# ShenhanQian/GaussianAvatars

Measured on AMD Instinct MI355X. Metric: frames/sec fwd+bwd @100k SH-3 splats 802x550, higher is better.
Workload: dtype f32; 1 GPU; BASELINE configs[2]: 100000 mesh-bound SH-3 splats (synthetic stand-in for media/306), 802x550 (HxW), select_mesh_by_timestep + render + L1-vs-white + backward, no optimiser step; splats=100000, width=550, height=802, sh_degree=3, scene=ellipsoid, splat_order=morton (io.spatial_sort: the loaders' default), num_rendered=2322054, num_binned=1851307, tile_culling=True, binding=fused, parallelism=one process, one GPU, 300 frames in turn; no collective

## Files before the change

### gaussianavatars_amd/_lib.py

```python
from __future__ import annotations

import ctypes as C
import os
from functools import partial
from typing import NamedTuple

_HERE = os.path.dirname(os.path.abspath(__file__))


def raw_stream(dev):
    import torch

    try:
        return torch._C._cuda_getCurrentRawStream(dev.index if dev.index is not None else torch.cuda.current_device())
    except AttributeError:
        return torch.cuda.current_stream(dev).cuda_stream


class _NoCtx:
    def __enter__(self):
        return None

    def __exit__(self, *a):
        return False
# ... 178 lines not shown

def gsr_profile_enable(on: bool) -> None:
    gsr().gsr_profile_enable(1 if on else 0)


def gsr_profile_read() -> dict:
    ms = (C.c_double * GSR_NUM_KERNELS)()
    n = (C.c_int64 * GSR_NUM_KERNELS)()
    rc = gsr().gsr_profile_read(ms, n)
    if rc != GSR_OK:
        raise RuntimeError(f"gsr_profile_read failed: {gsr().gsr_last_error().decode()}")
    return {gsr().gsr_kernel_name(i).decode(): (ms[i], n[i]) for i in range(GSR_NUM_KERNELS)}

def gsr_wait_stats():
    ms, n = C.c_double(), C.c_int64()
    gsr().gsr_wait_stats(C.byref(ms), C.byref(n))
    return ms.value, n.value


LIBS["gsr"] = LibSpec("gsr", GSR_LIB_PATH, GSR_SYMBOLS, GSR_ABI_VERSION)
_gsr = None


def gsr():
    global _gsr
    if _gsr is None:
        _gsr = _load(LIBS["gsr"])
    return _gsr


GAB_LIB_PATH = _lib_path("gab", "GAB_LIB")
GAB_FLAME_WS_FLOATS = 512
GAB_BIND_ROW_FLOATS = 20
_P = C.c_void_p


class GabRig(C.Structure):
    _fields_ = [("V", C.c_int32), ("n_shape", C.c_int32), ("n_expr", C.c_int32), ("v_template", _P), ("shapedirs", _P),
                ("posedirs", _P), ("J_regressor", _P), ("lbs_weights", _P), ("parents", C.c_int32 * 5)]


GAB_SYMBOLS = {
    "gab_abi_version": (C.c_int, []),
    "gab_last_error": (C.c_char_p, []),
    "gab_flame_forward": (C.c_int, [C.POINTER(GabRig)] + [_P] * 8 + [_P, _P, _P, _P]),
    "gab_flame_backward": (C.c_int, [C.POINTER(GabRig)] + [_P] * 8 + [_P, _P, _P, _P] + [_P] * 8 + [_P] +
                           [C.c_int32, C.POINTER(C.c_void_p), C.POINTER(C.c_int32), _P]),
    "gab_flame_prepared_floats": (C.c_int64, [C.POINTER(GabRig)]),
    "gab_flame_prepare": (C.c_int, [C.POINTER(GabRig), _P, _P, _P, _P]),
    "gab_flame_forward_prepared": (C.c_int, [C.POINTER(GabRig), _P] + [_P] * 6 + [_P, _P, _P, _P]),
    "gab_blend_sequence": (C.c_int, [C.POINTER(GabRig), _P, _P, C.c_int32, _P, _P]),
    "gab_flame_forward_sequence": (C.c_int, [C.POINTER(GabRig), _P, _P] + [_P] * 6 + [_P, _P, _P, _P]),
    "gab_flame_backward_prepared": (C.c_int, [C.POINTER(GabRig), _P] + [_P] * 4 + [_P, _P, _P] + [_P] * 6 + [_P] +
                                    [C.c_int32, C.POINTER(C.c_void_p), C.POINTER(C.c_int32), _P]),
    "gab_mesh_backward_prepared": (C.c_int, [C.POINTER(GabRig), _P] + [_P] * 4 + [_P, _P, _P, _P, _P] + [_P] * 5 + [_P] * 6 + [_P] +
                                   [C.c_int32, C.POINTER(C.c_void_p), C.POINTER(C.c_int32), _P]),
    "gab_face_frames_forward": (C.c_int, [C.c_int32, C.c_int32, _P, _P, C.c_int32, _P, _P, _P, _P, _P, _P]),
    "gab_face_frames_backward": (C.c_int, [C.c_int32, C.c_int32, _P, _P, C.c_int32, _P, _P, _P, _P, _P, C.c_int32, _P]),
    "gab_bind_forward": (C.c_int, [C.c_int32, C.c_int32, _P, _P, _P, _P, C.c_int32, _P, _P, _P, _P, _P, _P, _P, _P, _P, _P]),
    "gab_bind_backward": (C.c_int, [C.c_int32, C.c_int32, _P, _P, _P, _P, C.c_int32, _P, _P, _P, _P, _P, _P, _P, _P, _P, _P, _P, _P, _P, _P, _P]),
    "gab_bind_backward_csr": (C.c_int, [C.c_int32, C.c_int32] + [_P] * 22),
    "gab_bind_backward_faces": (C.c_int, [C.c_int32, _P, _P, _P, _P]),
    "gab_zero_buffers": (C.c_int, [C.c_int32, C.POINTER(C.c_void_p), C.POINTER(C.c_int32), _P]),
    "gab_feed_row": (C.c_int, [_P, C.c_int32, C.c_int32, _P, C.c_int32, _P, _P, _P]),
    **_profile_symbols("gab"),
}
GAB_ABI_VERSION = 5

LIBS["gab"] = LibSpec("gab", GAB_LIB_PATH, GAB_SYMBOLS, GAB_ABI_VERSION)
_gab = None


def gab():
    global _gab
    if _gab is None:
        _gab = _load(LIBS["gab"])
    return _gab


GLS_LIB_PATH = _lib_path("gls")
GLS_SYMBOLS = {
    "gls_abi_version": (C.c_int, []),
    "gls_last_error": (C.c_char_p, []),
    "gls_partial_floats": (C.c_int64, [C.c_int32] * 4),
    "gls_l1_ssim_forward": (C.c_int, [C.c_int32] * 4 + [_P, _P, C.c_float] + [_P] * 4),
    "gls_l1_ssim_backward": (C.c_int, [C.c_int32] * 4 + [_P] * 4 + [C.c_float, _P, _P]),
    "gls_l1_ssim_backward_split": (C.c_int, [C.c_int32] * 4 + [_P] * 5 + [C.c_int32, C.c_float, _P, _P]),
    "gls_l1_forward": (C.c_int, [C.c_int64, _P, _P, C.c_float, _P, _P, _P]),
    "gls_l1_forward_grad": (C.c_int, [C.c_int64, _P, _P, C.c_float, _P, _P, _P, _P]),
    "gls_l1_backward": (C.c_int, [C.c_int64, _P, _P, _P, C.c_float, _P, _P]),
    "gls_densification_stats": (C.c_int, [C.c_int32] + [_P] * 6),
    "gls_add_densification_stats": (C.c_int, [C.c_int32, _P, _P, C.c_int32, _P, _P, _P]),
    **_profile_symbols("gls"),
}
GLS_ABI_VERSION = 4

LIBS["gls"] = LibSpec("gls", GLS_LIB_PATH, GLS_SYMBOLS, GLS_ABI_VERSION)
_gls = None


# ... 323 lines not shown
```

### gaussianavatars_amd/binding.py

```python
from __future__ import annotations

import ctypes as C
import os

import torch

from . import _host, _lib


def _p(t):
    return None if t is None else t.data_ptr()


def _stream(dev):
    return _lib.raw_stream(dev)


def _chk(rc, what):
    if rc != 0:
        raise RuntimeError(f"{what} failed ({rc}): {_lib.gab_error()}")


def _need_cuda(t, name):
    if not t.is_cuda:
# ... 162 lines not shown
                                            _p(d_shape), _p(d_expr), _p(d_rot), _p(d_neck), _p(d_jaw), _p(d_eyes), _p(d_trans), _p(d_so),
                                            _p(scratch), 0, None, None, _stream(dev)), "gab_flame_backward")
        sh = ctx.shapes
        outs = [None, None if d_shape is None else d_shape.view(sh[0]), d_expr.view(sh[1]), d_rot.view(sh[2]), d_neck.view(sh[3]),
                d_jaw.view(sh[4]), d_eyes.view(sh[5]), d_trans.view(sh[6]), None if d_so is None else d_so.view(ctx.so_shape)]
        return tuple(outs)


def flame_forward(head, shape, expr, rotation, neck, jaw, eyes, translation, static_offset=None):
    return _FlameForward.apply(head, shape, expr, rotation, neck, jaw, eyes, translation, static_offset)


class _FlameForwardTimestep(torch.autograd.Function):

    _ROWS = ("expr", "rotation", "neck_pose", "jaw_pose", "eyes_pose", "translation")

    @staticmethod
    def forward(ctx, head, t, shape, expr, rotation, neck, jaw, eyes, translation, static_offset):
        ctx.set_materialize_grads(False)
        lib = _lib.gab()
        rig = _rig_struct(head)
        dev = head.v_template.device
        V = rig.V
        tabs = [_f32(x) for x in (expr, rotation, neck, jaw, eyes, translation)]
        T = tabs[0].shape[0]
        widths = [int(x.shape[1]) for x in tabs]
        if widths != [rig.n_expr, 3, 3, 3, 6, 3] or any(x.shape[0] != T for x in tabs) or not (0 <= t < T):
            raise RuntimeError("flame_forward_timestep: expected (T,n_expr),(T,3),(T,3),(T,3),(T,6),(T,3) tables and 0 <= t < T")
        sh = _f32(shape).reshape(-1)
        so = None if static_offset is None else _f32(static_offset).reshape(-1)
        rows = [x.data_ptr() + 4 * t * w for x, w in zip(tabs, widths)]
        verts = torch.empty((1, V, 3), dtype=torch.float32, device=dev)
        v_shaped = torch.empty((1, V, 3), dtype=torch.float32, device=dev)
        ws = torch.empty(_lib.GAB_FLAME_WS_FLOATS, dtype=torch.float32, device=dev)
        need = ctx.needs_input_grad
        ctx.prepared = _prepared_rig(head, rig, sh, so) if _use_prepared(head, need[2], so is not None and need[9]) else None
        seq = _sequence_table(head, rig, ctx.prepared, tabs[0]) if (ctx.prepared is not None and not any(need[2:])) else None
        with _lib.on_device(dev):
            if seq is not None:
                _chk(lib.gab_flame_forward_sequence(C.byref(rig), _p(ctx.prepared), seq.data_ptr() + 4 * t * 3 * V, *rows, _p(verts), _p(v_shaped),
                                                    _p(ws), _stream(dev)), "gab_flame_forward_sequence")
            elif ctx.prepared is not None:
                _chk(lib.gab_flame_forward_prepared(C.byref(rig), _p(ctx.prepared), *rows, _p(verts), _p(v_shaped), _p(ws), _stream(dev)),
                     "gab_flame_forward_prepared")
            else:
                _chk(lib.gab_flame_forward(C.byref(rig), _p(sh), *rows, _p(so), _p(verts), _p(v_shaped), _p(ws), _stream(dev)),
                     "gab_flame_forward")
        ctx.head, ctx.t, ctx.T, ctx.widths = head, t, T, widths
        ctx.has_so = so is not None
        ctx.shape_shape = shape.shape
        ctx.so_shape = None if static_offset is None else static_offset.shape
        ctx.keep = _Keep(sh, *tabs, *([so] if so is not None else []), v_shaped, ws)
        return verts, v_shaped

    @staticmethod
    def backward(ctx, g_verts, g_vshaped):
        lib = _lib.gab()
        rig = _rig_struct(ctx.head)
        saved = ctx.keep.get()
        sh, tabs = saved[0], list(saved[1:7])
        so = saved[7] if ctx.has_so else None
        v_shaped, ws = saved[-2], saved[-1]
        dev = v_shaped.device
        V, T, t, widths = rig.V, ctx.T, ctx.t, ctx.widths
        need = ctx.needs_input_grad
        f32 = dict(dtype=torch.float32, device=dev)
        tables = [torch.empty((T, w), **f32) for w in widths]
# ... 275 lines not shown
```

### gaussianavatars_amd/csrc/gaa_host.cpp

```cpp
#include <torch/extension.h>

#include <ATen/hip/impl/HIPGuardImplMasqueradingAsCUDA.h>
#include <c10/hip/HIPStream.h>
#include <dlfcn.h>
#include <torch/csrc/autograd/function.h>
#include <torch/csrc/autograd/functions/utils.h>

#include <atomic>
#include <map>
#include <mutex>
#include <tuple>

#include "../../include/gab.h"
#include "../../include/gls.h"
#include "../../include/gsr.h"

namespace {

using at::Tensor;
using torch::autograd::Node;
using torch::autograd::variable_list;

#define GAA_API(X)                                                                                                                      \
    X(gsr_abi_version) X(gsr_last_error) X(gsr_geom_layout) X(gsr_binning_layout) X(gsr_image_layout) X(gsr_forward_bound)             \
// ... 128 lines not shown
        Tensor scratch = empty_f32({3 * (int64_t)V}, v);
        Tensor gc = grad_f32(grads[2]), gR = grad_f32(grads[3]), gs = grad_f32(grads[4]), gq = grad_f32(grads[5]), gv = grad_f32(grads[0]);
        int rc = api.gab_mesh_backward_prepared(&p.rig, p.prepared.data_ptr<float>(), rows[1], rows[2], rows[3], rows[4], vs.data_ptr<float>(), ws.data_ptr<float>(),
                                                v.data_ptr<float>(), p.vf_begin.data_ptr<int32_t>(), p.vf_list.data_ptr<int32_t>(), fptr(gc), fptr(gR), fptr(gs), fptr(gq),
                                                fptr(gv), outp[0], outp[1], outp[2], outp[3], outp[4], outp[5], scratch.data_ptr<float>(), 6, zero_ptrs, zero_sizes, stream);
        TORCH_CHECK(rc == 0, "gab_mesh_backward_prepared failed (", rc, "): ", api.gab_last_error());
        variable_list out(6);
        for (int i = 0; i < 6; ++i)
            if (task_should_compute_output(i)) out[i] = tables[i];
        return out;
    }
    void release_variables() override {}
};

std::vector<Tensor> mesh_frames(const std::shared_ptr<MeshPlan>& plan, const Tensor& expr, const Tensor& rotation, const Tensor& neck, const Tensor& jaw,
                                const Tensor& eyes, const Tensor& translation, int64_t t)
{
    need_api();
    const MeshPlan& p = *plan;
    const Tensor* tabs[6] = {&expr, &rotation, &neck, &jaw, &eyes, &translation};
    const int64_t widths[6] = {p.rig.n_expr, 3, 3, 3, 6, 3};
    static const char* names[6] = {"expr", "rotation", "neck_pose", "jaw_pose", "eyes_pose", "translation"};
    const int64_t T = expr.dim() == 2 ? expr.size(0) : -1;
    TORCH_CHECK(T > 0 && t >= 0 && t < T, "flame_forward_timestep: expected (T,n_expr),(T,3),(T,3),(T,3),(T,6),(T,3) tables and 0 <= t < T");
    for (int i = 0; i < 6; ++i) {
        check_f32(*tabs[i], names[i]);
        TORCH_CHECK(tabs[i]->dim() == 2 && tabs[i]->size(0) == T && tabs[i]->size(1) == widths[i],
                    "flame_forward_timestep: expected (T,n_expr),(T,3),(T,3),(T,3),(T,6),(T,3) tables and 0 <= t < T");
    }
    const Tensor& like = p.prepared;
    DeviceGuard guard(like.device().index());
    void* stream = cur_stream(like);
    const int64_t V = p.rig.V, F = p.F;
    Tensor verts = empty_f32({1, V, 3}, like), v_shaped = empty_f32({1, V, 3}, like), ws = empty_f32({GAB_FLAME_WS_FLOATS}, like);
    Tensor center = empty_f32({F, 3}, like), R = empty_f32({F, 3, 3}, like), scale = empty_f32({F, 1}, like), quat = empty_f32({F, 4}, like);
    const float* rows[6];
    for (int i = 0; i < 6; ++i) rows[i] = tabs[i]->data_ptr<float>() + t * widths[i];
    int rc = api.gab_flame_forward_prepared(&p.rig, p.prepared.data_ptr<float>(), rows[0], rows[1], rows[2], rows[3], rows[4], rows[5], verts.data_ptr<float>(),
                                            v_shaped.data_ptr<float>(), ws.data_ptr<float>(), stream);
    TORCH_CHECK(rc == 0, "gab_flame_forward_prepared failed (", rc, "): ", api.gab_last_error());
    rc = api.gab_face_frames_forward((int32_t)V, (int32_t)F, verts.data_ptr<float>(), p.faces.data_ptr(), p.faces_i64, center.data_ptr<float>(), R.data_ptr<float>(),
                                     scale.data_ptr<float>(), quat.data_ptr<float>(), nullptr , stream);
    TORCH_CHECK(rc == 0, "gab_face_frames_forward failed (", rc, "): ", api.gab_last_error());
    if (any_requires_grad({expr, rotation, neck, jaw, eyes, translation})) {
        auto node = std::shared_ptr<MeshNode>(new MeshNode(), torch::autograd::deleteNode);
        node->set_next_edges(torch::autograd::collect_next_edges(expr, rotation, neck, jaw, eyes, translation));
        node->plan = plan;
        for (int i = 0; i < 6; ++i) {
            node->tabs[i] = Kept(*tabs[i]);
            node->widths[i] = widths[i];
        }
        node->verts = Kept(verts, true);
        node->v_shaped = Kept(v_shaped, true);
        node->ws = ws;
        node->t = t;
        node->T = T;
        torch::autograd::set_history({verts, v_shaped, center, R, scale, quat}, node);
    }
    return {verts, v_shaped, center, R, scale, quat};
}

struct Layouts {
    GsrGeomLayout geom;
    GsrImageLayout img;
};
std::mutex layout_mutex;
std::map<std::tuple<int64_t, int, int>, Layouts> layout_cache;
// ... 430 lines not shown
```

### gaussianavatars_amd/csrc/gab_kernels.hip

```cpp
#include <hip/hip_runtime.h>
#include <hip/amd_detail/amd_hip_unsafe_atomics.h>

#include "../../include/gab.h"
#include "launch_prof.h"
#include "lib_common.h"
#include "bind_math.h"
#include "wave_reduce.h"

namespace gab {

struct Rig {
    int V, n_shape, n_expr;
    const float* __restrict__ v_template;
    const float* __restrict__ shapedirs;
    const float* __restrict__ posedirs;
    const float* __restrict__ J_regressor;
    const float* __restrict__ lbs_weights;
    int parents[GAB_NUM_JOINTS];
};

constexpr int WS_J = 0;
constexpr int WS_R = 16;
constexpr int WS_PF = 64;
constexpr int WS_A = 128;
// ... 441 lines not shown
        for (int p = 0; p < GAB_POSE_FEATURES; ++p) {
            const float* row = rig.posedirs + (size_t)p * E + 3 * v;
            pf[p] = row[0] * gvp[0] + row[1] * gvp[1] + row[2] * gvp[2];
        }
    }
    const float vph[4] = {vp[0], vp[1], vp[2], ok ? 1.f : 0.f};
#pragma unroll
    for (int j = 0; j < GAB_NUM_JOINTS; ++j)
#pragma unroll
        for (int r = 0; r < 3; ++r)
#pragma unroll
            for (int c = 0; c < 4; ++c) {
                const float s = wave_sum_hi(w[j] * g[r] * vph[c]);
                if (lane == 63) red[wid][12 * j + 4 * r + c] = s;
            }
#pragma unroll
    for (int r = 0; r < 3; ++r) {
        const float s = wave_sum_hi(g[r]);
        if (lane == 63) red[wid][60 + r] = s;
    }
#pragma unroll
    for (int p = 0; p < GAB_POSE_FEATURES; ++p) {
        const float s = wave_sum_hi(pf[p]);
        if (lane == 63) red[wid][63 + p] = s;
    }
    __syncthreads();
    if (tid < 99) {
        const float s = (red[0][tid] + red[1][tid]) + (red[2][tid] + red[3][tid]);
        float* dst = tid < 60 ? &ws[WS_DA + tid] : (tid < 63 ? &ws[WS_DT + tid - 60] : &ws[WS_DPF + tid - 63]);
        unsafeAtomicAdd(dst, s);
    }
}

template <bool FLAME_TREE, int NT>
__device__ __forceinline__ void chain_bwd_body(Rig rig, float* __restrict__ ws, const float* __restrict__ rotation, const float* __restrict__ neck,
                            const float* __restrict__ jaw, const float* __restrict__ eyes, float* __restrict__ d_rotation,
                            float* __restrict__ d_neck, float* __restrict__ d_jaw, float* __restrict__ d_eyes,
                            float* __restrict__ d_translation, float* __restrict__ d_expr, float* __restrict__ d_shape,
                            const float* __restrict__ Mmat)
{
    __shared__ float sw[GAB_FLAME_WS_FLOATS];
    __shared__ float sdJ[16];
    for (int kk = threadIdx.x; kk < GAB_FLAME_WS_FLOATS; kk += NT) sw[kk] = ws[kk];
    __syncthreads();
    for (int kk = WS_DA + (int)threadIdx.x; kk < WS_DJ; kk += NT) ws[kk] = 0.f;
    if (!Mmat) {
        for (int kk = threadIdx.x; kk < rig.n_expr; kk += NT) d_expr[kk] = 0.f;
        if (d_shape)
            for (int kk = threadIdx.x; kk < rig.n_shape; kk += NT) d_shape[kk] = 0.f;
    }
    __shared__ float sdR[45];
    if (threadIdx.x == 0) {
    float J[15], R[45], Rg[45], tg[15];
#pragma unroll
    for (int k = 0; k < 15; ++k) J[k] = sw[WS_J + k];
#pragma unroll
    for (int k = 0; k < 45; ++k) R[k] = sw[WS_R + k];
    chain_forward<FLAME_TREE>(rig.parents, R, J, Rg, tg);
    float dRg[45], dtg[15], dJ[15], dR[45];
#pragma unroll
    for (int k = 0; k < 45; ++k) { dRg[k] = 0.f; dR[k] = 0.f; }
#pragma unroll
    for (int k = 0; k < 15; ++k) { dtg[k] = 0.f; dJ[k] = 0.f; }
#pragma unroll
    for (int i = 0; i < GAB_NUM_JOINTS; ++i) {
        const float* dA = sw + WS_DA + 12 * i;
#pragma unroll
        for (int r = 0; r < 3; ++r) {
            const float dAt = dA[4 * r + 3];
#pragma unroll
            for (int c = 0; c < 3; ++c) {
                dRg[9 * i + 3 * r + c] += dA[4 * r + c] - dAt * J[3 * i + c];
                dJ[3 * i + c] -= Rg[9 * i + 3 * r + c] * dAt;
            }
            dtg[3 * i + r] += dAt;
        }
    }
#pragma unroll
// ... 105 lines not shown
        if (c < nC) {
            const float* col = rig.shapedirs + (size_t)e0 * NB + c0 + c;
            int r = r0;
            for (; r + 8 <= r1; r += 8) {
                float x[8];
#pragma unroll
                for (int k = 0; k < 8; ++k) x[k] = col[(size_t)(r + k) * NB];
#pragma unroll
                for (int k = 0; k < 8; ++k) acc += x[k] * g[r + k];
            }
            for (; r < r1; ++r) acc += col[(size_t)r * NB] * g[r];
        }
        if (half == 1) part[cl] = acc;
        __syncthreads();
        if (half == 0 && c < nC) {
            const int l = c0 + c;
            float* dst = l < rig.n_shape ? d_shape + l : d_expr + (l - rig.n_shape);
            unsafeAtomicAdd(dst, acc + part[cl]);
        }
        __syncthreads();
    }
}
__global__ __launch_bounds__(256) void k_blend_bwd(Rig rig, const float* __restrict__ ws, const float* __restrict__ g_vs,
                                                    const float* __restrict__ dL_dv_shaped, float* __restrict__ d_static_offset,
                                                    float* __restrict__ d_shape, float* __restrict__ d_expr)
{
    blend_bwd_body(rig, ws, g_vs, dL_dv_shaped, d_static_offset, d_shape, d_expr, (int)blockIdx.x);
}
template <bool FLAME_TREE>
__global__ __launch_bounds__(256) void k_chain_blend_bwd(Rig rig, float* __restrict__ ws, const float* __restrict__ g_vs, const float* __restrict__ Mmat,
                                                          const float* __restrict__ rotation, const float* __restrict__ neck,
                                                          const float* __restrict__ jaw, const float* __restrict__ eyes,
                                                          float* __restrict__ d_rotation, float* __restrict__ d_neck, float* __restrict__ d_jaw,
                                                          float* __restrict__ d_eyes, float* __restrict__ d_translation, float* __restrict__ d_expr)
{
    if (blockIdx.x == 0)
        chain_bwd_body<FLAME_TREE, 256>(rig, ws, rotation, neck, jaw, eyes, d_rotation, d_neck, d_jaw, d_eyes, d_translation, d_expr, nullptr, Mmat);
    else
        blend_bwd_body(rig, nullptr, g_vs, nullptr, nullptr, nullptr, d_expr, (int)blockIdx.x - 1);
}

struct Vec3 { float x, y, z; };
__device__ __forceinline__ Vec3 operator-(Vec3 a, Vec3 b) { return {a.x - b.x, a.y - b.y, a.z - b.z}; }
__device__ __forceinline__ Vec3 operator+(Vec3 a, Vec3 b) { return {a.x + b.x, a.y + b.y, a.z + b.z}; }
__device__ __forceinline__ Vec3 operator*(Vec3 a, float s) { return {a.x * s, a.y * s, a.z * s}; }
__device__ __forceinline__ float dot(Vec3 a, Vec3 b) { return a.x * b.x + a.y * b.y + a.z * b.z; }
__device__ __forceinline__ Vec3 cross(Vec3 a, Vec3 b) { return {a.y * b.z - a.z * b.y, a.z * b.x - a.x * b.z, a.x * b.y - a.y * b.x}; }
__device__ __forceinline__ Vec3 ld3(const float* p, long long i) { return {p[3 * i], p[3 * i + 1], p[3 * i + 2]}; }

__device__ __forceinline__ long long index_at(const void* idx, int is64, long long i)
{
    return is64 ? ((const long long*)idx)[i] : (long long)((const int*)idx)[i];
}

struct Frame {
    Vec3 e1, e2, a0, a1, a2, n, m;
    float l1, ln, lm, d;
    bool c1, cn, cm;
};
__device__ __forceinline__ Frame make_frame(Vec3 v0, Vec3 v1, Vec3 v2)
{
    Frame f;
    const float eps = 1e-20f;
    f.e1 = v1 - v0;
    f.e2 = v2 - v0;
    float q = dot(f.e1, f.e1);
    f.c1 = q < eps; f.l1 = sqrtf(f.c1 ? eps : q);
    f.a0 = f.e1 * (1.f / f.l1);
    f.n = cross(f.a0, f.e2);
    q = dot(f.n, f.n);
// ... 98 lines not shown
        const float sg = fr.d > 0.f ? 1.f : (fr.d < 0.f ? -1.f : 0.f);
        g_a2 = g_a2 + fr.e2 * (gs * sg);
        g_e2 = g_e2 + fr.a2 * (gs * sg);
    }
    const Vec3 u = fr.a2 * -1.f;
    const Vec3 g_m = unit_bwd(g_a2 * -1.f, u, fr.lm, fr.cm);
    g_a1 = g_a1 + cross(fr.a0, g_m);
    g_a0 = g_a0 + cross(g_m, fr.a1);
    const Vec3 g_n = unit_bwd(g_a1, fr.a1, fr.ln, fr.cn);
    g_a0 = g_a0 + cross(fr.e2, g_n);
    g_e2 = g_e2 + cross(g_n, fr.a0);
    Vec3 g_e1 = unit_bwd(g_a0, fr.a0, fr.l1, fr.c1);
    if (!fr.c1) g_e1 = g_e1 + fr.a0 * g_l1;
    Vec3 gc = {0.f, 0.f, 0.f};
    if (d_center) gc = Vec3{d_center[3 * f], d_center[3 * f + 1], d_center[3 * f + 2]} * (1.f / 3.f);
    g0 = gc - g_e1 - g_e2; g1 = gc + g_e1; g2 = gc + g_e2;
}

__global__ __launch_bounds__(256) void k_face_frames_bwd(int F, const float* __restrict__ verts, const void* __restrict__ faces, int is64,
                                                          const float* __restrict__ d_center, const float* __restrict__ d_R,
                                                          const float* __restrict__ d_scaling, const float* __restrict__ d_quat,
                                                          float* __restrict__ d_verts)
{
    const int f = blockIdx.x * blockDim.x + threadIdx.x;
    if (f >= F) return;
    const long long i0 = index_at(faces, is64, 3ll * f), i1 = index_at(faces, is64, 3ll * f + 1), i2 = index_at(faces, is64, 3ll * f + 2);
    Vec3 g0, g1, g2;
    face_frame_bwd(f, ld3(verts, i0), ld3(verts, i1), ld3(verts, i2), d_center, d_R, d_scaling, d_quat, g0, g1, g2);
    unsafeAtomicAdd(&d_verts[3 * i0], g0.x); unsafeAtomicAdd(&d_verts[3 * i0 + 1], g0.y); unsafeAtomicAdd(&d_verts[3 * i0 + 2], g0.z);
    unsafeAtomicAdd(&d_verts[3 * i1], g1.x); unsafeAtomicAdd(&d_verts[3 * i1 + 1], g1.y); unsafeAtomicAdd(&d_verts[3 * i1 + 2], g1.z);
    unsafeAtomicAdd(&d_verts[3 * i2], g2.x); unsafeAtomicAdd(&d_verts[3 * i2 + 1], g2.y); unsafeAtomicAdd(&d_verts[3 * i2 + 2], g2.z);
}

#ifndef GAB_MESH_VPB
#define GAB_MESH_VPB 32
#endif
struct GatherSkinArgs {
    const float* v_shaped; float* ws;
    const float* verts;
    const int* vf_begin; const int4* vf_list;
    const float* d_center; const float* d_R; const float* d_scaling; const float* d_quat;
    const float* g_verts;
    float* g_vs;
};
__global__ __launch_bounds__(256) void k_gather_skin_bwd(Rig rig, GatherSkinArgs a, ZeroSpec zero)
{
    constexpr int VPB = GAB_MESH_VPB, ROWS = 3 * VPB;
    static_assert(VPB == 16 || VPB == 32 || VPB == 64, "a wave holds the workgroup's vertices");
    __shared__ float gv[ROWS];
    __shared__ float red[100];
    constexpr int PDN = GAB_POSE_FEATURES * ROWS, PDK = (PDN + 255) / 256;
    __shared__ float pd[GAB_POSE_FEATURES][ROWS];
    const int tid = threadIdx.x, lane = tid & 63, wid = __builtin_amdgcn_readfirstlane(tid >> 6);
    const int gid = blockIdx.x * 256 + tid;
    for (int b = 0; b < zero.count; ++b)
        for (int i = gid; i < zero.n[b]; i += (int)(gridDim.x * 256)) zero.p[b][i] = 0.f;
    const int vbase = blockIdx.x * VPB, vend = min(vbase + VPB, rig.V);
    const int E = 3 * rig.V;
    const int p0 = a.vf_begin[vbase], p1 = a.vf_begin[vend];
    float pdr[PDK];
#pragma unroll
    for (int i = 0; i < PDK; ++i) {
        const int k = tid + 256 * i, p = k / ROWS, c = k - p * ROWS;
        pdr[i] = (k < PDN && 3 * vbase + c < E) ? rig.posedirs[(size_t)p * E + 3 * vbase + c] : 0.f;
    }
    const int v = vbase + lane;
    const bool ok = lane < VPB && v < rig.V;
    float vs[3] = {0.f, 0.f, 0.f}, gx[3] = {0.f, 0.f, 0.f};
    float w[GAB_NUM_JOINTS] = {0.f, 0.f, 0.f, 0.f, 0.f};
    if (ok) {
#pragma unroll
        for (int k = 0; k < 3; ++k) { vs[k] = a.v_shaped[3 * v + k]; gx[k] = a.g_verts ? a.g_verts[3 * v + k] : 0.f; }
#pragma unroll
        for (int j = 0; j < GAB_NUM_JOINTS; ++j) w[j] = rig.lbs_weights[(size_t)v * GAB_NUM_JOINTS + j];
    }
    for (int k = tid; k < ROWS; k += 256) gv[k] = 0.f;
    __syncthreads();
    float tc[3] = {0.f, 0.f, 0.f};
    for (int p = p0 + tid; p < p1; p += 256) {
        const int4 e = a.vf_list[p];
        const int f = e.x >> 2, c = e.x & 3;
        Vec3 g0, g1, g2;
        face_frame_bwd(f, ld3(a.verts, e.y), ld3(a.verts, e.z), ld3(a.verts, e.w), a.d_center, a.d_R, a.d_scaling, a.d_quat, g0, g1, g2);
        const Vec3 g = c == 0 ? g0 : (c == 1 ? g1 : g2);
        const int vl = (c == 0 ? e.y : (c == 1 ? e.z : e.w)) - vbase;
        atomicAdd(&gv[3 * vl], g.x); atomicAdd(&gv[3 * vl + 1], g.y); atomicAdd(&gv[3 * vl + 2], g.z);
        if (a.d_center) {
#pragma unroll
            for (int r = 0; r < 3; ++r) tc[r] += a.d_center[3 * f + r] * (1.0f / 3.0f);
        }
    }
    __shared__ float tcs[4][3];
#pragma unroll
    for (int r = 0; r < 3; ++r) {
        const float s = wave_sum_hi(tc[r]);
        if (lane == 63) tcs[wid][r] = s;
    }
#pragma unroll
    for (int i = 0; i < PDK; ++i) {
        const int k = tid + 256 * i;
        if (k < PDN) (&pd[0][0])[k] = pdr[i];
    }
    __syncthreads();
    float g[3] = {0.f, 0.f, 0.f}, vp[3] = {0.f, 0.f, 0.f}, T[12], gvp[3] = {0.f, 0.f, 0.f};
    float pf[GAB_POSE_FEATURES];
#pragma unroll
    for (int p = 0; p < GAB_POSE_FEATURES; ++p) pf[p] = 0.f;
    if (ok) {
        float po[3] = {0.f, 0.f, 0.f};
#pragma unroll
        for (int p = 0; p < GAB_POSE_FEATURES; ++p) {
            const float f = a.ws[WS_PF + p];
            po[0] += f * pd[p][3 * lane]; po[1] += f * pd[p][3 * lane + 1]; po[2] += f * pd[p][3 * lane + 2];
        }
#pragma unroll
        for (int k = 0; k < 3; ++k) vp[k] = po[k] + vs[k];
#pragma unroll
        for (int k = 0; k < 12; ++k) T[k] = 0.f;
#pragma unroll
        for (int j = 0; j < GAB_NUM_JOINTS; ++j)
#pragma unroll
            for (int k = 0; k < 12; ++k) T[k] += w[j] * a.ws[WS_A + 12 * j + k];
#pragma unroll
        for (int k = 0; k < 3; ++k) g[k] = gv[3 * lane + k] + gx[k];
#pragma unroll
        for (int c = 0; c < 3; ++c) gvp[c] = T[c] * g[0] + T[4 + c] * g[1] + T[8 + c] * g[2];
#pragma unroll
        for (int p = 0; p < GAB_POSE_FEATURES; ++p) pf[p] = pd[p][3 * lane] * gvp[0] + pd[p][3 * lane + 1] * gvp[1] + pd[p][3 * lane + 2] * gvp[2];
        if (wid == 0) { a.g_vs[3 * v] = gvp[0]; a.g_vs[3 * v + 1] = gvp[1]; a.g_vs[3 * v + 2] = gvp[2]; }
    }
    const float vph[4] = {vp[0], vp[1], vp[2], ok ? 1.f : 0.f};
#pragma unroll
    for (int j = 0; j < GAB_NUM_JOINTS; ++j) {
        if (wid != (j >> 1)) continue;
#pragma unroll
        for (int r = 0; r < 3; ++r)
#pragma unroll
            for (int c = 0; c < 4; ++c) {
                const float s = wave_sum_hi(w[j] * g[r] * vph[c]);
                if (lane == 63) red[12 * j + 4 * r + c] = s;
            }
    }
    if (wid == 2) {
#pragma unroll
        for (int r = 0; r < 3; ++r) {
            const float s = wave_sum_hi(gx[r]);
            if (lane == 63) red[60 + r] = s + ((tcs[0][r] + tcs[1][r]) + (tcs[2][r] + tcs[3][r]));
        }
    }
#pragma unroll
    for (int p = 0; p < GAB_POSE_FEATURES; ++p) {
        if (wid != (p < 9 ? 2 : 3)) continue;
        const float s = wave_sum_hi(pf[p]);
        if (lane == 63) red[63 + p] = s;
    }
    __syncthreads();
    if (tid < 99) {
        float* dst = tid < 60 ? &a.ws[WS_DA + tid] : (tid < 63 ? &a.ws[WS_DT + tid - 60] : &a.ws[WS_DPF + tid - 63]);
        unsafeAtomicAdd(dst, red[tid]);
    }
}

using bindm::qmul;
using bindm::qconj;
using bindm::qnorm_clamped;

__global__ __launch_bounds__(256) void k_bind(int N, const float* __restrict__ xyz, const float* __restrict__ log_scaling,
                                               const float* __restrict__ rotation, const void* __restrict__ binding, int is64,
                                               const float* __restrict__ fc, const float* __restrict__ fR, const float* __restrict__ fs,
                                               const float* __restrict__ fq, float* __restrict__ out_xyz, float* __restrict__ out_scaling,
                                               float* __restrict__ out_rotation, const float* __restrict__ opacity_logit,
                                               float* __restrict__ out_opacity)
{
    const int i = blockIdx.x * blockDim.x + threadIdx.x;
    if (i >= N) return;
    if (opacity_logit) out_opacity[i] = bindm::sigmoid(opacity_logit[i]);
    const long long f = index_at(binding, is64, i);
    const float s = fs[f];
    float w[3];
    bindm::world_xyz(fR + 9 * f, s, fc + 3 * f, xyz[3 * i], xyz[3 * i + 1], xyz[3 * i + 2], w);
    for (int r = 0; r < 3; ++r) out_xyz[3 * i + r] = w[r];
    for (int k = 0; k < 3; ++k) out_scaling[3 * i + k] = bindm::world_scaling(log_scaling[3 * i + k], s);
    reinterpret_cast<float4*>(out_rotation)[i] = bindm::world_rotation(reinterpret_cast<const float4*>(fq)[f], reinterpret_cast<const float4*>(rotation)[i]);
}

__global__ __launch_bounds__(256) void k_bind_bwd(int N, const float* __restrict__ xyz, const float* __restrict__ log_scaling,
                                                   const float* __restrict__ rotation, const void* __restrict__ binding, int is64,
                                                   const float* __restrict__ fR, const float* __restrict__ fs, const float* __restrict__ fq,
                                                   const float* __restrict__ g_xyz, const float* __restrict__ g_scaling,
                                                   const float* __restrict__ g_rot, float* __restrict__ d_xyz,
                                                   float* __restrict__ d_log_scaling, float* __restrict__ d_rotation, float* __restrict__ d_face, int F,
                                                   const float* __restrict__ out_opacity, const float* __restrict__ g_opacity,
                                                   float* __restrict__ d_opacity_logit)
// ... 529 lines not shown
}

int gab_flame_backward_prepared(const GabRig* rig_, const float* prepared, const float* rotation, const float* neck, const float* jaw,
                                const float* eyes, const float* v_shaped, float* ws, const float* dL_dverts, float* d_expr,
                                float* d_rotation, float* d_neck, float* d_jaw, float* d_eyes, float* d_translation, float* scratch,
                                int32_t zero_count, float* const* zero_buffers_host, const int32_t* zero_sizes_host, void* stream_)
{
    if (zero_count < 0 || zero_count > 7 || (zero_count > 0 && (!zero_buffers_host || !zero_sizes_host)))
        return fail(GAB_E_ARG, "gab_flame_backward_prepared: 0..7 zero-fill buffers");
    gab::Rig rig;
    if (int rc = to_rig(rig_, &rig)) return rc;
    if (!prepared || !rotation || !neck || !jaw || !eyes || !v_shaped || !ws || !dL_dverts || !d_expr || !d_rotation || !d_neck || !d_jaw ||
        !d_eyes || !d_translation || !scratch)
        return fail(GAB_E_ARG, "gab_flame_backward_prepared: NULL buffer");
    gab::ZeroSpec zs;
    bool covers_expr = false;
    for (int i = 0; i < 8; ++i) {
        zs.p[i] = i < zero_count ? zero_buffers_host[i] : nullptr;
        zs.n[i] = i < zero_count ? zero_sizes_host[i] : 0;
        if (i < zero_count && (zs.n[i] < 0 || (zs.n[i] > 0 && !zs.p[i]))) return fail(GAB_E_ARG, "gab_flame_backward_prepared: bad zero-fill buffer %d", i);
        if (i < zero_count && d_expr >= zs.p[i] && d_expr + rig.n_expr <= zs.p[i] + zs.n[i]) covers_expr = true;
    }
    zs.count = zero_count;
    if (!covers_expr) { zs.p[zs.count] = d_expr; zs.n[zs.count] = rig.n_expr; ++zs.count; }
    hipStream_t st = (hipStream_t)stream_;
    const int E = 3 * rig.V;
    PROF_LAUNCH(gab::k_skin_bwd, dim3((rig.V + 255) / 256), dim3(256), 0, st, rig, ws, v_shaped, dL_dverts, scratch, zs);
    LAUNCH_CHECK(GAB_E_HIP, "launch of k_skin_bwd failed");
    const float* Mmat = prepared + gab::prep_joint_offset(rig.V) + 16;
    const int blocks = 1 + (E + GAB_BLEND_BWD_ROWS - 1) / GAB_BLEND_BWD_ROWS;
    const bool flame_tree = rig.parents[1] == 0 && rig.parents[2] == 1 && rig.parents[3] == 1 && rig.parents[4] == 1;
    if (flame_tree)
        PROF_LAUNCH(gab::k_chain_blend_bwd<true>, dim3(blocks), dim3(256), 0, st, rig, ws, (const float*)scratch, Mmat, rotation, neck, jaw, eyes,
                           d_rotation, d_neck, d_jaw, d_eyes, d_translation, d_expr);
    else
        PROF_LAUNCH(gab::k_chain_blend_bwd<false>, dim3(blocks), dim3(256), 0, st, rig, ws, (const float*)scratch, Mmat, rotation, neck, jaw, eyes,
                           d_rotation, d_neck, d_jaw, d_eyes, d_translation, d_expr);
    LAUNCH_CHECK(GAB_E_HIP, "launch of k_chain_blend_bwd failed");
    return GAB_OK;
}

int gab_mesh_backward_prepared(const GabRig* rig_, const float* prepared, const float* rotation, const float* neck, const float* jaw,
                               const float* eyes, const float* v_shaped, float* ws, const float* verts, const int32_t* vf_begin,
                               const int32_t* vf_list, const float* d_center, const float* d_orien_mat, const float* d_scaling,
                               const float* d_orien_quat, const float* dL_dverts, float* d_expr, float* d_rotation, float* d_neck,
                               float* d_jaw, float* d_eyes, float* d_translation, float* scratch, int32_t zero_count,
                               float* const* zero_buffers_host, const int32_t* zero_sizes_host, void* stream_)
{
    if (zero_count < 0 || zero_count > 7 || (zero_count > 0 && (!zero_buffers_host || !zero_sizes_host)))
        return fail(GAB_E_ARG, "gab_mesh_backward_prepared: 0..7 zero-fill buffers");
    gab::Rig rig;
    if (int rc = to_rig(rig_, &rig)) return rc;
    if (!prepared || !rotation || !neck || !jaw || !eyes || !v_shaped || !ws || !verts || !vf_begin || !vf_list || !d_expr || !d_rotation ||
        !d_neck || !d_jaw || !d_eyes || !d_translation || !scratch)
        return fail(GAB_E_ARG, "gab_mesh_backward_prepared: NULL buffer");
    gab::ZeroSpec zs;
    bool covers_expr = false;
    for (int i = 0; i < 8; ++i) {
        zs.p[i] = i < zero_count ? zero_buffers_host[i] : nullptr;
        zs.n[i] = i < zero_count ? zero_sizes_host[i] : 0;
        if (i < zero_count && (zs.n[i] < 0 || (zs.n[i] > 0 && !zs.p[i]))) return fail(GAB_E_ARG, "gab_mesh_backward_prepared: bad zero-fill buffer %d", i);
        if (i < zero_count && d_expr >= zs.p[i] && d_expr + rig.n_expr <= zs.p[i] + zs.n[i]) covers_expr = true;
    }
    zs.count = zero_count;
    if (!covers_expr) { zs.p[zs.count] = d_expr; zs.n[zs.count] = rig.n_expr; ++zs.count; }
    gab::GatherSkinArgs a;
    a.v_shaped = v_shaped; a.ws = ws; a.verts = verts;
    a.vf_begin = vf_begin; a.vf_list = reinterpret_cast<const int4*>(vf_list);
    a.d_center = d_center; a.d_R = d_orien_mat; a.d_scaling = d_scaling; a.d_quat = d_orien_quat; a.g_verts = dL_dverts;
    a.g_vs = scratch;
    hipStream_t st = (hipStream_t)stream_;
    PROF_LAUNCH(gab::k_gather_skin_bwd, dim3((rig.V + GAB_MESH_VPB - 1) / GAB_MESH_VPB), dim3(256), 0, st, rig, a, zs);
    LAUNCH_CHECK(GAB_E_HIP, "launch of k_gather_skin_bwd failed");
    const int E = 3 * rig.V;
    const float* Mmat = prepared + gab::prep_joint_offset(rig.V) + 16;
    const int blocks = 1 + (E + GAB_BLEND_BWD_ROWS - 1) / GAB_BLEND_BWD_ROWS;
    const bool flame_tree = rig.parents[1] == 0 && rig.parents[2] == 1 && rig.parents[3] == 1 && rig.parents[4] == 1;
    if (flame_tree)
        PROF_LAUNCH(gab::k_chain_blend_bwd<true>, dim3(blocks), dim3(256), 0, st, rig, ws, (const float*)scratch, Mmat, rotation, neck, jaw, eyes,
                           d_rotation, d_neck, d_jaw, d_eyes, d_translation, d_expr);
    else
        PROF_LAUNCH(gab::k_chain_blend_bwd<false>, dim3(blocks), dim3(256), 0, st, rig, ws, (const float*)scratch, Mmat, rotation, neck, jaw, eyes,
                           d_rotation, d_neck, d_jaw, d_eyes, d_translation, d_expr);
    LAUNCH_CHECK(GAB_E_HIP, "launch of k_chain_blend_bwd failed");
    return GAB_OK;
}

int gab_face_frames_forward(int32_t V, int32_t F, const float* verts, const void* faces, int32_t is64, float* center, float* orien_mat,
                            float* scaling, float* orien_quat, float* d_verts_zeroed, void* stream_)
{
    if (V <= 0 || F < 0) return fail(GAB_E_ARG, "bad sizes");
    if (F == 0) {
        if (d_verts_zeroed) HIP_TRY(hipMemsetAsync(d_verts_zeroed, 0, (size_t)V * 3 * sizeof(float), (hipStream_t)stream_));
        return GAB_OK;
    }
    if (!verts || !faces || !center || !orien_mat || !scaling || !orien_quat) return fail(GAB_E_ARG, "gab_face_frames_forward: NULL buffer");
    PROF_LAUNCH(gab::k_face_frames, dim3((F + 255) / 256), dim3(256), 0, (hipStream_t)stream_, F, verts, faces, is64, center, orien_mat,
                       scaling, orien_quat, d_verts_zeroed, 3 * V);
    LAUNCH_CHECK(GAB_E_HIP, "launch of k_face_frames failed");
    return GAB_OK;
}

int gab_face_frames_backward(int32_t V, int32_t F, const float* verts, const void* faces, int32_t is64, const float* d_center,
                             const float* d_orien_mat, const float* d_scaling, const float* d_orien_quat, float* d_verts,
                             int32_t d_verts_is_zero, void* stream_)
{
    if (V <= 0 || F < 0) return fail(GAB_E_ARG, "bad sizes");
    if (!d_verts) return fail(GAB_E_ARG, "d_verts is NULL");
    hipStream_t st = (hipStream_t)stream_;
    if (!d_verts_is_zero) HIP_TRY(hipMemsetAsync(d_verts, 0, (size_t)V * 3 * sizeof(float), st));
    if (F == 0) return GAB_OK;
    if (!verts || !faces) return fail(GAB_E_ARG, "gab_face_frames_backward: NULL buffer");
    PROF_LAUNCH(gab::k_face_frames_bwd, dim3((F + 255) / 256), dim3(256), 0, st, F, verts, faces, is64, d_center, d_orien_mat, d_scaling,
                       d_orien_quat, d_verts);
    LAUNCH_CHECK(GAB_E_HIP, "launch of k_face_frames_bwd failed");
    return GAB_OK;
// ... 118 lines not shown
```

### include/gab.h

```cpp
#ifndef GAB_H
#define GAB_H

#include <stddef.h>
#include <stdint.h>

#ifdef __cplusplus
extern "C" {
#endif

#define GAB_ABI_VERSION 5
#define GAB_OK 0
#define GAB_E_ARG (-1)
#define GAB_E_HIP (-2)

#define GAB_NUM_JOINTS 5
#define GAB_POSE_FEATURES 36
#define GAB_FLAME_WS_FLOATS 512

typedef struct GabRig {
    int32_t V;
    int32_t n_shape;
    int32_t n_expr;
    const float* v_template;
    const float* shapedirs;
    const float* posedirs;
    const float* J_regressor;
    const float* lbs_weights;
    int32_t parents[GAB_NUM_JOINTS];
} GabRig;

int gab_abi_version(void);
const char* gab_last_error(void);

int gab_flame_forward(const GabRig* rig, const float* shape, const float* expr, const float* rotation,
                      const float* neck, const float* jaw, const float* eyes , const float* translation,
                      const float* static_offset ,
                      float* verts , float* v_shaped , float* ws , void* stream);

int gab_flame_backward(const GabRig* rig, const float* shape, const float* expr, const float* rotation,
                       const float* neck, const float* jaw, const float* eyes, const float* translation,
                       const float* static_offset, const float* v_shaped, float* ws,
                       const float* dL_dverts, const float* dL_dv_shaped,
                       float* d_shape, float* d_expr, float* d_rotation, float* d_neck, float* d_jaw, float* d_eyes,
                       float* d_translation, float* d_static_offset, float* scratch,
                       int32_t zero_count, float* const* zero_buffers_host, const int32_t* zero_sizes_host, void* stream);

int64_t gab_flame_prepared_floats(const GabRig* rig);
int gab_flame_prepare(const GabRig* rig, const float* shape, const float* static_offset , float* prepared, void* stream);
int gab_flame_forward_prepared(const GabRig* rig, const float* prepared, const float* expr, const float* rotation, const float* neck,
                               const float* jaw, const float* eyes , const float* translation,
// ... 65 lines not shown
```

Before: 4001 frames/s.

## Replace mesh backward global atomics with per-block rows and deterministic reduction

The gather-skin backward kernel now writes each block's 99 partial sums (joint transforms, translation, pose features) to a per-block row in an enlarged workspace instead of atomically adding into ws. The chain backward kernel reduces these rows with float4 loads in a fixed order. Separately, per-vertex gradient accumulation in shared memory moves from shared atomics to a staged segmented sum over a CSR vertex-begin table. This removes global and shared atomic contention and makes the sums deterministic, at the cost of a larger workspace, extra syncs and serial per-vertex loops.

```diff
diff --git a/gaussianavatars_amd/_lib.py b/gaussianavatars_amd/_lib.py
--- a/gaussianavatars_amd/_lib.py
+++ b/gaussianavatars_amd/_lib.py
@@ -234,6 +234,12 @@
 GAB_LIB_PATH = _lib_path("gab", "GAB_LIB")
 GAB_FLAME_WS_FLOATS = 512
 GAB_BIND_ROW_FLOATS = 20
+GAB_MESH_ROW_FLOATS = 100
+GAB_MESH_VPB = 32
+
+
+def gab_mesh_ws_floats(V: int) -> int:
+    return GAB_FLAME_WS_FLOATS + GAB_MESH_ROW_FLOATS * ((V + GAB_MESH_VPB - 1) // GAB_MESH_VPB)
 _P = C.c_void_p
 
 
@@ -267,7 +273,7 @@
     "gab_feed_row": (C.c_int, [_P, C.c_int32, C.c_int32, _P, C.c_int32, _P, _P, _P]),
     **_profile_symbols("gab"),
 }
-GAB_ABI_VERSION = 5
+GAB_ABI_VERSION = 6
 
 LIBS["gab"] = LibSpec("gab", GAB_LIB_PATH, GAB_SYMBOLS, GAB_ABI_VERSION)
 _gab = None
diff --git a/gaussianavatars_amd/binding.py b/gaussianavatars_amd/binding.py
--- a/gaussianavatars_amd/binding.py
+++ b/gaussianavatars_amd/binding.py
@@ -218,7 +218,7 @@
         rows = [x.data_ptr() + 4 * t * w for x, w in zip(tabs, widths)]
         verts = torch.empty((1, V, 3), dtype=torch.float32, device=dev)
         v_shaped = torch.empty((1, V, 3), dtype=torch.float32, device=dev)
-        ws = torch.empty(_lib.GAB_FLAME_WS_FLOATS, dtype=torch.float32, device=dev)
+        ws = torch.empty(_lib.gab_mesh_ws_floats(V), dtype=torch.float32, device=dev)
         need = ctx.needs_input_grad
         ctx.prepared = _prepared_rig(head, rig, sh, so) if _use_prepared(head, need[2], so is not None and need[9]) else None
         seq = _sequence_table(head, rig, ctx.prepared, tabs[0]) if (ctx.prepared is not None and not any(need[2:])) else None
diff --git a/gaussianavatars_amd/csrc/gaa_host.cpp b/gaussianavatars_amd/csrc/gaa_host.cpp
--- a/gaussianavatars_amd/csrc/gaa_host.cpp
+++ b/gaussianavatars_amd/csrc/gaa_host.cpp
@@ -184,7 +184,7 @@
     DeviceGuard guard(like.device().index());
     void* stream = cur_stream(like);
     const int64_t V = p.rig.V, F = p.F;
-    Tensor verts = empty_f32({1, V, 3}, like), v_shaped = empty_f32({1, V, 3}, like), ws = empty_f32({GAB_FLAME_WS_FLOATS}, like);
+    Tensor verts = empty_f32({1, V, 3}, like), v_shaped = empty_f32({1, V, 3}, like), ws = empty_f32({GAB_MESH_WS_FLOATS(V)}, like);
     Tensor center = empty_f32({F, 3}, like), R = empty_f32({F, 3, 3}, like), scale = empty_f32({F, 1}, like), quat = empty_f32({F, 4}, like);
     const float* rows[6];
     for (int i = 0; i < 6; ++i) rows[i] = tabs[i]->data_ptr<float>() + t * widths[i];
diff --git a/gaussianavatars_amd/csrc/gab_kernels.hip b/gaussianavatars_amd/csrc/gab_kernels.hip
--- a/gaussianavatars_amd/csrc/gab_kernels.hip
+++ b/gaussianavatars_amd/csrc/gab_kernels.hip
@@ -497,18 +497,50 @@
     }
 }
 
+constexpr int ROWSUM_GROUPS = 10, ROWSUM_DEPTH = 20, ROW_F4 = GAB_MESH_ROW_FLOATS / 4;
 template <bool FLAME_TREE, int NT>
 __device__ __forceinline__ void chain_bwd_body(Rig rig, float* __restrict__ ws, const float* __restrict__ rotation, const float* __restrict__ neck,
                             const float* __restrict__ jaw, const float* __restrict__ eyes, float* __restrict__ d_rotation,
                             float* __restrict__ d_neck, float* __restrict__ d_jaw, float* __restrict__ d_eyes,
                             float* __restrict__ d_translation, float* __restrict__ d_expr, float* __restrict__ d_shape,
-                            const float* __restrict__ Mmat)
+                            const float* __restrict__ Mmat, const float* __restrict__ rows = nullptr, int n_rows = 0)
 {
     __shared__ float sw[GAB_FLAME_WS_FLOATS];
     __shared__ float sdJ[16];
     for (int kk = threadIdx.x; kk < GAB_FLAME_WS_FLOATS; kk += NT) sw[kk] = ws[kk];
+    if (NT == 256 && rows) {
+        static_assert(ROWSUM_GROUPS * ROW_F4 <= 256 && ROW_F4 * 4 == GAB_MESH_ROW_FLOATS, "one thread per (row group, float4 of a row)");
+        __shared__ float4 part[ROWSUM_GROUPS][ROW_F4];
+        const int g = (int)threadIdx.x / ROW_F4, c = (int)threadIdx.x - g * ROW_F4;
+        if (g < ROWSUM_GROUPS) {
+            const float4* r4 = reinterpret_cast<const float4*>(rows);
+            float4 acc = make_float4(0.f, 0.f, 0.f, 0.f);
+            for (int r0 = g; r0 < n_rows; r0 += ROWSUM_GROUPS * ROWSUM_DEPTH) {
+                float4 x[ROWSUM_DEPTH];
+#pragma unroll
+                for (int i = 0; i < ROWSUM_DEPTH; ++i) {
+                    const int r = r0 + ROWSUM_GROUPS * i;
+                    x[i] = r < n_rows ? r4[(size_t)r * ROW_F4 + c] : make_float4(0.f, 0.f, 0.f, 0.f);
+                }
+#pragma unroll
+                for (int i = 0; i < ROWSUM_DEPTH; ++i) { acc.x += x[i].x; acc.y += x[i].y; acc.z += x[i].z; acc.w += x[i].w; }
+            }
+            part[g][c] = acc;
+        }
+        __syncthreads();
+        if (threadIdx.x < 99) {
+            const float* pp = reinterpret_cast<const float*>(&part[0][0]) + threadIdx.x;
+            float p[ROWSUM_GROUPS];
+#pragma unroll
+            for (int i = 0; i < ROWSUM_GROUPS; ++i) p[i] = pp[i * GAB_MESH_ROW_FLOATS];
+            const int k = threadIdx.x;
+            sw[k < 60 ? WS_DA + k : (k < 63 ? WS_DT + k - 60 : WS_DPF + k - 63)] =
+                (((p[0] + p[1]) + (p[2] + p[3])) + ((p[4] + p[5]) + (p[6] + p[7]))) + (p[8] + p[9]);
+        }
+    }
     __syncthreads();
-    for (int kk = WS_DA + (int)threadIdx.x; kk < WS_DJ; kk += NT) ws[kk] = 0.f;
+    if (!(NT == 256 && rows))
+        for (int kk = WS_DA + (int)threadIdx.x; kk < WS_DJ; kk += NT) ws[kk] = 0.f;
     if (!Mmat) {
         for (int kk = threadIdx.x; kk < rig.n_expr; kk += NT) d_expr[kk] = 0.f;
         if (d_shape)
@@ -680,10 +712,12 @@
                                                           const float* __restrict__ rotation, const float* __restrict__ neck,
                                                           const float* __restrict__ jaw, const float* __restrict__ eyes,
                                                           float* __restrict__ d_rotation, float* __restrict__ d_neck, float* __restrict__ d_jaw,
-                                                          float* __restrict__ d_eyes, float* __restrict__ d_translation, float* __restrict__ d_expr)
+                                                          float* __restrict__ d_eyes, float* __restrict__ d_translation, float* __restrict__ d_expr,
+                                                          const float* __restrict__ rows, int n_rows)
 {
     if (blockIdx.x == 0)
-        chain_bwd_body<FLAME_TREE, 256>(rig, ws, rotation, neck, jaw, eyes, d_rotation, d_neck, d_jaw, d_eyes, d_translation, d_expr, nullptr, Mmat);
+        chain_bwd_body<FLAME_TREE, 256>(rig, ws, rotation, neck, jaw, eyes, d_rotation, d_neck, d_jaw, d_eyes, d_translation, d_expr, nullptr, Mmat, rows,
+                                        n_rows);
     else
         blend_bwd_body(rig, nullptr, g_vs, nullptr, nullptr, nullptr, d_expr, (int)blockIdx.x - 1);
 }
@@ -848,9 +882,6 @@
     unsafeAtomicAdd(&d_verts[3 * i2], g2.x); unsafeAtomicAdd(&d_verts[3 * i2 + 1], g2.y); unsafeAtomicAdd(&d_verts[3 * i2 + 2], g2.z);
 }
 
-#ifndef GAB_MESH_VPB
-#define GAB_MESH_VPB 32
-#endif
 struct GatherSkinArgs {
     const float* v_shaped; float* ws;
     const float* verts;
@@ -858,6 +889,7 @@
     const float* d_center; const float* d_R; const float* d_scaling; const float* d_quat;
     const float* g_verts;
     float* g_vs;
+    float* rows;
 };
 __global__ __launch_bounds__(256) void k_gather_skin_bwd(Rig rig, GatherSkinArgs a, ZeroSpec zero)
 {
@@ -869,6 +901,7 @@
     __shared__ float pd[GAB_POSE_FEATURES][ROWS];
     const int tid = threadIdx.x, lane = tid & 63, wid = __builtin_amdgcn_readfirstlane(tid >> 6);
     const int gid = blockIdx.x * 256 + tid;
+    const float *wpf = a.ws + WS_PF, *wA = a.ws + WS_A;
     for (int b = 0; b < zero.count; ++b)
         for (int i = gid; i < zero.n[b]; i += (int)(gridDim.x * 256)) zero.p[b][i] = 0.f;
     const int vbase = blockIdx.x * VPB, vend = min(vbase + VPB, rig.V);
@@ -891,19 +924,34 @@
         for (int j = 0; j < GAB_NUM_JOINTS; ++j) w[j] = rig.lbs_weights[(size_t)v * GAB_NUM_JOINTS + j];
     }
     for (int k = tid; k < ROWS; k += 256) gv[k] = 0.f;
+    __shared__ int vb[VPB + 1];
+    __shared__ float cg[3][256];
+    if (tid <= VPB) vb[tid] = a.vf_begin[min(vbase + tid, rig.V)];
     __syncthreads();
     float tc[3] = {0.f, 0.f, 0.f};
-    for (int p = p0 + tid; p < p1; p += 256) {
-        const int4 e = a.vf_list[p];
-        const int f = e.x >> 2, c = e.x & 3;
-        Vec3 g0, g1, g2;
-        face_frame_bwd(f, ld3(a.verts, e.y), ld3(a.verts, e.z), ld3(a.verts, e.w), a.d_center, a.d_R, a.d_scaling, a.d_quat, g0, g1, g2);
-        const Vec3 g = c == 0 ? g0 : (c == 1 ? g1 : g2);
-        const int vl = (c == 0 ? e.y : (c == 1 ? e.z : e.w)) - vbase;
-        atomicAdd(&gv[3 * vl], g.x); atomicAdd(&gv[3 * vl + 1], g.y); atomicAdd(&gv[3 * vl + 2], g.z);
-        if (a.d_center) {
-#pragma unroll
-            for (int r = 0; r < 3; ++r) tc[r] += a.d_center[3 * f + r] * (1.0f / 3.0f);
+    for (int base = p0; base < p1; base += 256) {
+        if (base != p0) __syncthreads();
+        const int p = base + tid;
+        Vec3 g = {0.f, 0.f, 0.f};
+        if (p < p1) {
+            const int4 e = a.vf_list[p];
+            const int f = e.x >> 2, c = e.x & 3;
+            Vec3 g0, g1, g2;
+            face_frame_bwd(f, ld3(a.verts, e.y), ld3(a.verts, e.z), ld3(a.verts, e.w), a.d_center, a.d_R, a.d_scaling, a.d_quat, g0, g1, g2);
+            g = c == 0 ? g0 : (c == 1 ? g1 : g2);
+            if (a.d_center) {
+#pragma unroll
+                for (int r = 0; r < 3; ++r) tc[r] += a.d_center[3 * f + r] * (1.0f / 3.0f);
+            }
+        }
+        cg[0][tid] = g.x; cg[1][tid] = g.y; cg[2][tid] = g.z;
+        __syncthreads();
+        if (tid < ROWS) {
+            const int vl = tid / 3, k = tid - 3 * vl;
+            const int q1 = min(vb[vl + 1], base + 256) - base;
+            float s = gv[tid];
+            for (int q = max(vb[vl], base) - base; q < q1; ++q) s += cg[k][q];
+            gv[tid] = s;
         }
     }
     __shared__ float tcs[4][3];
@@ -926,7 +974,7 @@
         float po[3] = {0.f, 0.f, 0.f};
 #pragma unroll
         for (int p = 0; p < GAB_POSE_FEATURES; ++p) {
-            const float f = a.ws[WS_PF + p];
+            const float f = wpf[p];
             po[0] += f * pd[p][3 * lane]; po[1] += f * pd[p][3 * lane + 1]; po[2] += f * pd[p][3 * lane + 2];
         }
 #pragma unroll
@@ -936,7 +984,7 @@
 #pragma unroll
         for (int j = 0; j < GAB_NUM_JOINTS; ++j)
 #pragma unroll
-            for (int k = 0; k < 12; ++k) T[k] += w[j] * a.ws[WS_A + 12 * j + k];
+            for (int k = 0; k < 12; ++k) T[k] += w[j] * wA[12 * j + k];
 #pragma unroll
         for (int k = 0; k < 3; ++k) g[k] = gv[3 * lane + k] + gx[k];
 #pragma unroll
@@ -971,10 +1019,7 @@
         if (lane == 63) red[63 + p] = s;
     }
     __syncthreads();
-    if (tid < 99) {
-        float* dst = tid < 60 ? &a.ws[WS_DA + tid] : (tid < 63 ? &a.ws[WS_DT + tid - 60] : &a.ws[WS_DPF + tid - 63]);
-        unsafeAtomicAdd(dst, red[tid]);
-    }
+    if (tid < 99) a.rows[(size_t)blockIdx.x * GAB_MESH_ROW_FLOATS + tid] = red[tid];
 }
 
 using bindm::qmul;
@@ -1570,10 +1615,10 @@
     const bool flame_tree = rig.parents[1] == 0 && rig.parents[2] == 1 && rig.parents[3] == 1 && rig.parents[4] == 1;
     if (flame_tree)
         PROF_LAUNCH(gab::k_chain_blend_bwd<true>, dim3(blocks), dim3(256), 0, st, rig, ws, (const float*)scratch, Mmat, rotation, neck, jaw, eyes,
-                           d_rotation, d_neck, d_jaw, d_eyes, d_translation, d_expr);
+                           d_rotation, d_neck, d_jaw, d_eyes, d_translation, d_expr, (const float*)nullptr, 0);
     else
         PROF_LAUNCH(gab::k_chain_blend_bwd<false>, dim3(blocks), dim3(256), 0, st, rig, ws, (const float*)scratch, Mmat, rotation, neck, jaw, eyes,
-                           d_rotation, d_neck, d_jaw, d_eyes, d_translation, d_expr);
+                           d_rotation, d_neck, d_jaw, d_eyes, d_translation, d_expr, (const float*)nullptr, 0);
     LAUNCH_CHECK(GAB_E_HIP, "launch of k_chain_blend_bwd failed");
     return GAB_OK;
 }
@@ -1607,8 +1652,11 @@
     a.vf_begin = vf_begin; a.vf_list = reinterpret_cast<const int4*>(vf_list);
     a.d_center = d_center; a.d_R = d_orien_mat; a.d_scaling = d_scaling; a.d_quat = d_orien_quat; a.g_verts = dL_dverts;
     a.g_vs = scratch;
+    if ((uintptr_t)ws & 15) return fail(GAB_E_ARG, "gab_mesh_backward_prepared: ws must be 16-byte aligned");
+    const int n_rows = (rig.V + GAB_MESH_VPB - 1) / GAB_MESH_VPB;
+    a.rows = ws + GAB_FLAME_WS_FLOATS;
     hipStream_t st = (hipStream_t)stream_;
-    PROF_LAUNCH(gab::k_gather_skin_bwd, dim3((rig.V + GAB_MESH_VPB - 1) / GAB_MESH_VPB), dim3(256), 0, st, rig, a, zs);
+    PROF_LAUNCH(gab::k_gather_skin_bwd, dim3(n_rows), dim3(256), 0, st, rig, a, zs);
     LAUNCH_CHECK(GAB_E_HIP, "launch of k_gather_skin_bwd failed");
     const int E = 3 * rig.V;
     const float* Mmat = prepared + gab::prep_joint_offset(rig.V) + 16;
@@ -1616,10 +1664,10 @@
     const bool flame_tree = rig.parents[1] == 0 && rig.parents[2] == 1 && rig.parents[3] == 1 && rig.parents[4] == 1;
     if (flame_tree)
         PROF_LAUNCH(gab::k_chain_blend_bwd<true>, dim3(blocks), dim3(256), 0, st, rig, ws, (const float*)scratch, Mmat, rotation, neck, jaw, eyes,
-                           d_rotation, d_neck, d_jaw, d_eyes, d_translation, d_expr);
+                           d_rotation, d_neck, d_jaw, d_eyes, d_translation, d_expr, (const float*)a.rows, n_rows);
     else
         PROF_LAUNCH(gab::k_chain_blend_bwd<false>, dim3(blocks), dim3(256), 0, st, rig, ws, (const float*)scratch, Mmat, rotation, neck, jaw, eyes,
-                           d_rotation, d_neck, d_jaw, d_eyes, d_translation, d_expr);
+                           d_rotation, d_neck, d_jaw, d_eyes, d_translation, d_expr, (const float*)a.rows, n_rows);
     LAUNCH_CHECK(GAB_E_HIP, "launch of k_chain_blend_bwd failed");
     return GAB_OK;
 }
diff --git a/include/gab.h b/include/gab.h
--- a/include/gab.h
+++ b/include/gab.h
@@ -8,7 +8,7 @@
 extern "C" {
 #endif
 
-#define GAB_ABI_VERSION 5
+#define GAB_ABI_VERSION 6
 #define GAB_OK 0
 #define GAB_E_ARG (-1)
 #define GAB_E_HIP (-2)
@@ -16,6 +16,11 @@
 #define GAB_NUM_JOINTS 5
 #define GAB_POSE_FEATURES 36
 #define GAB_FLAME_WS_FLOATS 512
+#define GAB_MESH_ROW_FLOATS 100
+#ifndef GAB_MESH_VPB
+#define GAB_MESH_VPB 32
+#endif
+#define GAB_MESH_WS_FLOATS(V) (GAB_FLAME_WS_FLOATS + GAB_MESH_ROW_FLOATS * (((V) + GAB_MESH_VPB - 1) / GAB_MESH_VPB))
 
 typedef struct GabRig {
     int32_t V;
```

After: 3998 frames/s. Within noise of the previous version (-0.1%).
